# lucidrains/e2-tts-pytorch

Hardware: NVIDIA H100
Metric: mel-frames/sec E2TTS fwd+bwd (d512 depth8 L1024) (higher is better)
Workload: dtype bf16

## Files before the change

e2-tts-pytorch_b200/csrc/attn_tc.cu:

```cuda
#include <type_traits>

#include "common.cuh"
#include "ptx.cuh"

namespace b200 {

constexpr int TQ = 128, TKV = 128;
constexpr int TILE16 = 128 * 64 * 2;
constexpr int TILE8 = 64 * 64 * 2;
constexpr float LOG2E_F = 1.4426950408889634f;

struct AttnTcP {
    const unsigned int* maskbits;
    int mask_words;
    const float* gate;
    __nv_bfloat16 *o, *og;
    float* lse;
    int B, H, Np, nkv;
    float scale_over_clamp, clamp, dropout_p, keep_scale;
    unsigned int drop_thresh;
    int drop_stride;
    unsigned long long seed;
    const unsigned long long* seed_dev;
    float scale, scale_log2e;
};

__device__ __forceinline__ float tanh_approx(float x) {
    float y;
    asm("tanh.approx.f32 %0, %1;" : "=f"(y) : "f"(x));
    return y;
}
constexpr float TANH_POLY_MAX = 0.5f;
__device__ __forceinline__ float2 tanh_poly2(float2 x) {
    const float2 x2 = fmul2(x, x);
    float2 q = ffma2(x2, make_float2(62.f / 2835.f, 62.f / 2835.f), make_float2(-17.f / 315.f, -17.f / 315.f));
    q = ffma2(q, x2, make_float2(2.f / 15.f, 2.f / 15.f));
    q = ffma2(q, x2, make_float2(-1.f / 3.f, -1.f / 3.f));
    q = ffma2(q, x2, make_float2(1.f, 1.f));
    return fmul2(x, q);
}
__device__ __forceinline__ float ex2_approx(float x) {
    float y;
    asm("ex2.approx.ftz.f32 %0, %1;" : "=f"(y) : "f"(x));
    return y;
}

__global__ void attn_maskbits_kernel(const unsigned char* mask, unsigned int* bits, int B, int Np, int words) {
    const int w = blockIdx.x * blockDim.x + threadIdx.x;
    if (w >= B * words) return;
    const int b = w / words, w0 = (w % words) * 32;
    unsigned int v = 0;
    for (int i = 0; i < 32; ++i) {
        const int n = w0 + i;
        if (n < Np && (!mask || mask[(size_t)b * Np + n])) v |= 1u << i;
    }
    bits[w] = v;
}

constexpr int KV_STAGES = 3;

template <bool UNCLAMPED, int DH>
__global__ void __launch_bounds__(384, 1)
attn_fwd_wgmma_kernel(const __grid_constant__ CUtensorMap tmQ, const __grid_constant__ CUtensorMap tmK, const __grid_constant__ CUtensorMap tmV,
                      const AttnTcP p) {
    extern __shared__ uint8_t smem_raw[];
    uint8_t* smem = smem_raw + ((1024u - (smem_u32(smem_raw) & 1023u)) & 1023u);
    constexpr int NA = DH / 64;
    uint8_t* sQ = smem;
    uint8_t* sK = sQ + NA * TILE16;
    uint8_t* sV = sK + KV_STAGES * NA * TILE8;
    uint64_t* bars = reinterpret_cast<uint64_t*>(sV + KV_STAGES * NA * TILE8);
    uint64_t* q_full = bars;
    uint64_t* kv_full = bars + 1;
    uint64_t* kv_empty = bars + 4;

    const int wg = threadIdx.x >> 7;
    const int qt = blockIdx.x, hh = blockIdx.y, b = blockIdx.z;
    const int bh = b * p.H + hh;
    const int q0 = qt * TQ;
    const int nkv = (p.Np + 63) / 64;

    if (threadIdx.x == 0) {
        tma_prefetch_desc(&tmQ); tma_prefetch_desc(&tmK); tma_prefetch_desc(&tmV);
        mbar_init(q_full, 1);
        for (int i = 0; i < KV_STAGES; ++i) { mbar_init(&kv_full[i], 1); mbar_init(&kv_empty[i], 2); }
        fence_barrier_init();
    }
    __syncthreads();

    if (wg == 0) {
        regs_dealloc<40>();
        if (threadIdx.x == 0) {
            const int row_base = bh * p.Np;
            mbar_arrive_expect_tx(q_full, NA * TILE16);
#pragma unroll
            for (int a = 0; a < NA; ++a) tma_load_2d(sQ + a * TILE16, &tmQ, q_full, 64 * a, row_base + q0);
            int st = 0;
            uint32_t ph = 0;
            for (int j = 0; j < nkv; ++j) {
                mbar_wait(&kv_empty[st], ph ^ 1);
                mbar_arrive_expect_tx(&kv_full[st], 2 * NA * TILE8);
#pragma unroll
                for (int a = 0; a < NA; ++a) {
                    tma_load_2d(sK + (st * NA + a) * TILE8, &tmK, &kv_full[st], 64 * a, row_base + j * 64);
                    tma_load_2d(sV + (st * NA + a) * TILE8, &tmV, &kv_full[st], 64 * a, row_base + j * 64);
                }
                if (++st == KV_STAGES) { st = 0; ph ^= 1; }
            }
        }
        return;
    }

    regs_alloc<232>();
    const int cw = wg - 1, t = threadIdx.x & 127, lane = t & 31, wq = t >> 5;
    const int cq = 2 * (lane & 3);
    const int r0 = cw * 64 + wq * 16 + (lane >> 2);
    const unsigned int* mb = p.maskbits + (size_t)b * p.mask_words;
    const uint32_t seedmix = seed_mix32(p.seed + (p.seed_dev ? __ldg(p.seed_dev) : 0ull));
    unsigned long long drop_row[2];
#pragma unroll
    for (int i = 0; i < 2; ++i) drop_row[i] = ((unsigned long long)bh * p.Np + (unsigned long long)(q0 + r0 + 8 * i)) * (unsigned long long)p.drop_stride;
    const float2 soc2 = make_float2(p.scale_over_clamp, p.scale_over_clamp);
    const float2 cl2 = make_float2(p.clamp * LOG2E_F, p.clamp * LOG2E_F);
    const float soc = p.scale_over_clamp, soc2s = soc * soc;
    const float k1 = soc * p.clamp * LOG2E_F, k3 = k1 * soc2s * (-1.f / 3.f), k5 = k1 * soc2s * soc2s * (2.f / 15.f),
                k7 = k1 * soc2s * soc2s * soc2s * (-17.f / 315.f), k9 = k1 * soc2s * soc2s * soc2s * soc2s * (62.f / 2835.f);
    const float lim5 = 0.15f / fabsf(soc), lim9 = TANH_POLY_MAX / fabsf(soc);
    const uint32_t thr32 = drop_thresh32(p.drop_thresh);
    float l[2] = {0.f, 0.f};
    float m[2] = {-INFINITY, -INFINITY};
    float o[NA][32];
#pragma unroll
    for (int a = 0; a < NA; ++a)
#pragma unroll
        for (int i = 0; i < 32; ++i) o[a][i] = 0.f;

    mbar_wait(q_full, 0);
    const uint64_t qdesc = make_smem_desc_sw128(smem_u32(sQ + cw * TILE8), 16, 1024);
    int st = 0;
    uint32_t ph = 0;
    for (int j = 0; j < nkv; ++j) {
        mbar_wait(&kv_full[st], ph);
        float s[32];
        fence_regs(s);
        wgmma_fence();
        const uint64_t kdesc = make_smem_desc_sw128(smem_u32(sK + st * NA * TILE8), 16, 1024);
#pragma unroll
        for (int k = 0; k < DH / 16; ++k)
            wgmma_ss_n64<0, 0>(s, qdesc + (uint64_t)((k >> 2) * (TILE16 >> 4) + (k & 3) * 2), kdesc + (uint64_t)((k >> 2) * (TILE8 >> 4) + (k & 3) * 2),
                               k > 0 ? 1u : 0u);
        wgmma_commit();
        wgmma_wait<0>();
        fence_regs(s);
        if constexpr (UNCLAMPED) {
            const unsigned int mw0 = mb[2 * j], mw1 = mb[2 * j + 1];
            if ((mw0 & mw1) != 0xffffffffu) {
#pragma unroll
                for (int g = 0; g < 8; ++g) {
                    const unsigned int w = g < 4 ? mw0 : mw1;
                    const int bit = (8 * g + cq) & 31;
#pragma unroll
                    for (int i = 0; i < 2; ++i) {
                        if (!((w >> bit) & 1u)) s[4 * g + 2 * i] = -INFINITY;
                        if (!((w >> (bit + 1)) & 1u)) s[4 * g + 2 * i + 1] = -INFINITY;
                    }
                }
            }
#pragma unroll
            for (int i = 0; i < 2; ++i) {
                float tm = m[i];
#pragma unroll
                for (int g = 0; g < 8; ++g) tm = fmaxf(tm, fmaxf(s[4 * g + 2 * i], s[4 * g + 2 * i + 1]));
                tm = fmaxf(tm, __shfl_xor_sync(0xffffffffu, tm, 1));
                tm = fmaxf(tm, __shfl_xor_sync(0xffffffffu, tm, 2));
                const float mt = tm == -INFINITY ? 0.f : tm;
                const float alpha = ex2_approx((m[i] - mt) * p.scale_log2e);
                const float nm = -mt * p.scale_log2e;
                m[i] = tm;
                float ls = 0.f;
#pragma unroll
                for (int g = 0; g < 8; ++g) {
#pragma unroll
                    for (int a = 0; a < NA; ++a) {
                        o[a][4 * g + 2 * i] *= alpha;
                        o[a][4 * g + 2 * i + 1] *= alpha;
                    }
                    s[4 * g + 2 * i] = ex2_approx(__fmaf_rn(s[4 * g + 2 * i], p.scale_log2e, nm));
                    s[4 * g + 2 * i + 1] = ex2_approx(__fmaf_rn(s[4 * g + 2 * i + 1], p.scale_log2e, nm));
                    ls += s[4 * g + 2 * i] + s[4 * g + 2 * i + 1];
                }
                l[i] = __fmaf_rn(l[i], alpha, ls);
            }
        } else {
            float amax = 0.f;
#pragma unroll
            for (int i = 0; i < 32; ++i) amax = fmaxf(amax, fabsf(s[i]));
            if (__all_sync(0xffffffffu, amax <= lim5)) {
#pragma unroll
                for (int i = 0; i < 32; i += 2) {
                    const float2 x = make_float2(s[i], s[i + 1]);
                    const float2 x2 = fmul2(x, x);
                    float2 q = ffma2(x2, make_float2(k5, k5), make_float2(k3, k3));
                    q = ffma2(q, x2, make_float2(k1, k1));
                    const float2 y = fmul2(x, q);
                    s[i] = ex2_approx(y.x);
                    s[i + 1] = ex2_approx(y.y);
                }
            } else if (__all_sync(0xffffffffu, amax <= lim9)) {
#pragma unroll
                for (int i = 0; i < 32; i += 2) {
                    const float2 x = make_float2(s[i], s[i + 1]);
                    const float2 x2 = fmul2(x, x);
                    float2 q = ffma2(x2, make_float2(k9, k9), make_float2(k7, k7));
                    q = ffma2(q, x2, make_float2(k5, k5));
                    q = ffma2(q, x2, make_float2(k3, k3));
                    q = ffma2(q, x2, make_float2(k1, k1));
                    const float2 y = fmul2(x, q);
                    s[i] = ex2_approx(y.x);
                    s[i + 1] = ex2_approx(y.y);
                }
            } else {
#pragma unroll
                for (int i = 0; i < 32; ++i) {
                    const float x = s[i], x2 = x * x;
                    const float yp = x * __fmaf_rn(__fmaf_rn(__fmaf_rn(__fmaf_rn(k9, x2, k7), x2, k5), x2, k3), x2, k1);
                    const float y = fabsf(x) <= lim9 ? yp : tanh_approx(x * soc) * cl2.x;
                    s[i] = ex2_approx(y);
                }
            }
            const unsigned int mw0 = mb[2 * j], mw1 = mb[2 * j + 1];
            if ((mw0 & mw1) != 0xffffffffu) {
#pragma unroll
                for (int g = 0; g < 8; ++g) {
                    const unsigned int w = g < 4 ? mw0 : mw1;
                    const int bit = (8 * g + cq) & 31;
#pragma unroll
                    for (int i = 0; i < 2; ++i) {
                        if (!((w >> bit) & 1u)) s[4 * g + 2 * i] = 0.f;
                        if (!((w >> (bit + 1)) & 1u)) s[4 * g + 2 * i + 1] = 0.f;
                    }
                }
            }
#pragma unroll
            for (int g = 0; g < 8; ++g)
#pragma unroll
                for (int i = 0; i < 2; ++i) l[i] += s[4 * g + 2 * i] + s[4 * g + 2 * i + 1];
        }
        if (p.dropout_p > 0.f) {
#pragma unroll
            for (int g = 0; g < 8; ++g)
#pragma unroll
                for (int i = 0; i < 2; ++i) {
                    const DropWords h = drop_words(seedmix, (uint32_t)((drop_row[i] + (unsigned long long)(j * 64 + 8 * g + cq)) >> 1));
                    s[4 * g + 2 * i] = (h.a >= thr32) ? s[4 * g + 2 * i] : 0.f;
                    s[4 * g + 2 * i + 1] = (h.b >= thr32) ? s[4 * g + 2 * i + 1] : 0.f;
                }
        }
#pragma unroll
        for (int a = 0; a < NA; ++a) fence_regs(o[a]);
        wgmma_fence();
        const uint64_t vdesc = make_smem_desc_sw128(smem_u32(sV + st * NA * TILE8), 64 * 128, 1024);
#pragma unroll
        for (int kk = 0; kk < 4; ++kk) {
            const uint32_t a[4] = {pack_bf16(s[8 * kk], s[8 * kk + 1]), pack_bf16(s[8 * kk + 2], s[8 * kk + 3]),
                                   pack_bf16(s[8 * kk + 4], s[8 * kk + 5]), pack_bf16(s[8 * kk + 6], s[8 * kk + 7])};
#pragma unroll
            for (int na = 0; na < NA; ++na) wgmma_rs_n64<1>(o[na], a, vdesc + (uint64_t)(na * (TILE8 >> 4) + kk * 128), 1u);
        }
        wgmma_commit();
        wgmma_wait<0>();
#pragma unroll
        for (int a = 0; a < NA; ++a) fence_regs(o[a]);
        if (t == 0) mbar_arrive(&kv_empty[st]);
        if (++st == KV_STAGES) { st = 0; ph ^= 1; }
    }
#pragma unroll
    for (int i = 0; i < 2; ++i) {
        float lt = l[i];
        lt += __shfl_xor_sync(0xffffffffu, lt, 1);
        lt += __shfl_xor_sync(0xffffffffu, lt, 2);
        const int qi = q0 + r0 + 8 * i;
        if (qi >= p.Np) continue;
        const float inv = lt > 0.f ? p.keep_scale / lt : 0.f;
        const float gt = p.gate ? p.gate[((size_t)b * p.Np + qi) * p.H + hh] : 1.f;
        __nv_bfloat16* orow = p.o + ((size_t)bh * p.Np + qi) * DH;
        __nv_bfloat16* grow = p.og + ((size_t)b * p.Np + qi) * (size_t)(p.H * DH) + hh * DH;
#pragma unroll
        for (int a = 0; a < NA; ++a)
#pragma unroll
            for (int g = 0; g < 8; ++g) {
                const uint32_t u = pack_bf16(o[a][4 * g + 2 * i] * inv, o[a][4 * g + 2 * i + 1] * inv);
                *reinterpret_cast<uint32_t*>(orow + 64 * a + 8 * g + cq) = u;
                *reinterpret_cast<uint32_t*>(grow + 64 * a + 8 * g + cq) = pack_bf16(bf16_lo(u) * gt, bf16_hi(u) * gt);
            }
        if ((lane & 3) == 0) {
            if constexpr (UNCLAMPED) p.lse[(size_t)bh * p.Np + qi] = __fmaf_rn(m[i], p.scale, logf(lt));
            else p.lse[(size_t)bh * p.Np + qi] = logf(lt);
        }
    }
}

struct AttnBwdTcP {
    const unsigned int* maskbits; int mask_words;
    const float *lse, *delta;
    __nv_bfloat16 *dk, *dv;
    int B, H, Np, nq;
    float scale, scale_over_clamp, clamp, dropout_p, keep_scale;
    unsigned int drop_thresh; int drop_stride;
    unsigned long long seed;
    const unsigned long long* seed_dev;
    float scale_log2e;
};
constexpr int QDO_STAGES = 3, TQB = 64;
constexpr int BAR_DS_FULL = 3, BAR_DS_FREE = 5;

struct AttnPrepP {
    const float* gate;
    const __nv_bfloat16* o;
    int B, H, Np;
    const __nv_bfloat16* dog;
    float* dgate;
    __nv_bfloat16* dO_out;
    float* delta_out;
};
template <int DH>
__global__ void __launch_bounds__(256) attn_bwd_prep_kernel(const AttnPrepP p) {
    constexpr int LANES = DH / 8, LOG2_LANES = DH == 64 ? 3 : 4;
    static_assert(LANES == 1 << LOG2_LANES, "head dim 64 or 128");
    const long long gidx = (long long)blockIdx.x * 256 + threadIdx.x;
    const long long rowid = gidx >> LOG2_LANES;
    const int c = (int)(gidx & (LANES - 1));
    const long long total = (long long)p.B * p.H * p.Np;
    const bool ok = rowid < total;
    float dot = 0.f, gt = 1.f;
    long long b = 0, hh = 0, n = 0;
    if (ok) {
        n = rowid % p.Np; hh = (rowid / p.Np) % p.H; b = rowid / ((long long)p.Np * p.H);
        const uint4 dg = *reinterpret_cast<const uint4*>(p.dog + ((size_t)b * p.Np + n) * (size_t)(p.H * DH) + hh * DH + c * 8);
        const uint4 ov = *reinterpret_cast<const uint4*>(p.o + (size_t)rowid * DH + c * 8);
        gt = p.gate ? p.gate[((size_t)b * p.Np + n) * p.H + hh] : 1.f;
        const uint32_t dgv[4] = {dg.x, dg.y, dg.z, dg.w}, ovv[4] = {ov.x, ov.y, ov.z, ov.w};
        uint32_t w[4];
#pragma unroll
        for (int i = 0; i < 4; ++i) {
            const float a0 = bf16_lo(dgv[i]), a1 = bf16_hi(dgv[i]);
            dot += a0 * bf16_lo(ovv[i]) + a1 * bf16_hi(ovv[i]);
            w[i] = pack_bf16(a0 * gt, a1 * gt);
        }
        *reinterpret_cast<uint4*>(p.dO_out + (size_t)rowid * DH + c * 8) = make_uint4(w[0], w[1], w[2], w[3]);
    }
#pragma unroll
    for (int m = 1; m < LANES; m <<= 1) dot += __shfl_xor_sync(0xffffffffu, dot, m);
    if (ok && c == 0) {
        p.delta_out[rowid] = dot * gt;
        if (p.dgate) p.dgate[((size_t)b * p.Np + n) * p.H + hh] = dot;
    }
}
// ... 521 lines not shown
    const PFN_encodeTiled2 enc = tensor_map_encoder();
    B200_REQUIRE(enc, "cuTensorMapEncodeTiled entry point not available");
    B200_REQUIRE((reinterpret_cast<uintptr_t>(ptr) & 15) == 0, "attention: operand not 16-byte aligned");
    cuuint64_t gdim[2] = {(cuuint64_t)dh, (cuuint64_t)rows};
    cuuint64_t gstride[1] = {(cuuint64_t)dh * 2};
    cuuint32_t box[2] = {64, (cuuint32_t)box_rows};
    cuuint32_t estr[2] = {1, 1};
    CUresult r = enc(m, CU_TENSOR_MAP_DATA_TYPE_BFLOAT16, 2, const_cast<void*>(ptr), gdim, gstride, box, estr, CU_TENSOR_MAP_INTERLEAVE_NONE,
                     CU_TENSOR_MAP_SWIZZLE_128B, CU_TENSOR_MAP_L2_PROMOTION_L2_256B, CU_TENSOR_MAP_FLOAT_OOB_FILL_NONE);
    B200_REQUIRE(r == CUDA_SUCCESS, "cuTensorMapEncodeTiled failed (%d)", (int)r);
    return 0;
}

static int make_dq_map(CUtensorMap* m, float* dq, int BH, int Np, int dh) {
    const PFN_encodeTiled2 enc = tensor_map_encoder();
    B200_REQUIRE(enc, "cuTensorMapEncodeTiled entry point not available");
    B200_REQUIRE((reinterpret_cast<uintptr_t>(dq) & 15) == 0, "attn_bwd: dq not 16-byte aligned");
    cuuint64_t gdim[3] = {(cuuint64_t)dh, (cuuint64_t)Np, (cuuint64_t)BH};
    cuuint64_t gstride[2] = {dh * sizeof(float), (cuuint64_t)Np * dh * sizeof(float)};
    cuuint32_t box[3] = {32, TQB, 1};
    cuuint32_t estr[3] = {1, 1, 1};
    CUresult r = enc(m, CU_TENSOR_MAP_DATA_TYPE_FLOAT32, 3, dq, gdim, gstride, box, estr, CU_TENSOR_MAP_INTERLEAVE_NONE,
                     CU_TENSOR_MAP_SWIZZLE_128B, CU_TENSOR_MAP_L2_PROMOTION_L2_256B, CU_TENSOR_MAP_FLOAT_OOB_FILL_NONE);
    B200_REQUIRE(r == CUDA_SUCCESS, "cuTensorMapEncodeTiled (dq) failed (%d)", (int)r);
    return 0;
}

}

using namespace b200;

extern "C" size_t b200_attn_workspace_bytes(int32_t B, int32_t Np) {
    const int words = ((Np + 127) / 128) * 4;
    return (size_t)B * words * sizeof(unsigned int);
}

extern "C" int b200_attn_maskbits(const uint8_t* keymask, void* ws_maskbits, int32_t B, int32_t Np, b200_stream_t stream) {
    B200_REQUIRE(ws_maskbits && B > 0 && Np > 0, "attn_maskbits: bad arguments");
    const int words = ((Np + TKV - 1) / TKV) * 4;
    attn_maskbits_kernel<<<(B * words + 127) / 128, 128, 0, reinterpret_cast<cudaStream_t>(stream)>>>(
        keymask, reinterpret_cast<unsigned int*>(ws_maskbits), B, Np, words);
    return check_launch("attn_maskbits_kernel");
}

extern "C" int b200_attn_fwd(const b200_attn_fwd_args* a, b200_stream_t stream) {
    cudaStream_t st = reinterpret_cast<cudaStream_t>(stream);
    B200_REQUIRE(a && a->q && a->k && a->v && a->o && a->og && a->lse && a->ws_maskbits, "attn_fwd: null pointer");
    B200_REQUIRE(a->dim_head == 64 || a->dim_head == 128, "attn_fwd: dim_head must be 64 or 128 (got %d)", a->dim_head);
    B200_REQUIRE(a->B > 0 && a->H > 0 && a->Np > 0 && a->B <= 65535 && a->H <= 65535, "attn_fwd: bad shape");
    if (a->unclamped) {
        B200_REQUIRE(a->softclamp == 0.f, "attn_fwd: unclamped attention needs softclamp == 0 (got %g)", a->softclamp);
    } else {
        B200_REQUIRE(a->softclamp > 0.f, "attn_fwd: softclamp value must be > 0, or set unclamped for attention without the logit soft-clamp");
    }
    B200_REQUIRE(a->dropout_p >= 0.f && a->dropout_p < 1.f, "attn_fwd: dropout must be in [0,1)");
    B200_REQUIRE(a->softclamp <= 64.f, "attn_fwd: softclamp %g > 64: the clamped wgmma kernel exponentiates the clamped logits without a "
                 "running maximum, which needs exp(+-softclamp) well inside fp32 / bf16 range (the reference uses 50)", a->softclamp);
    AttnTcP p{};
    p.nkv = (a->Np + TKV - 1) / TKV;
    p.mask_words = p.nkv * 4;
    p.maskbits = reinterpret_cast<const unsigned int*>(a->ws_maskbits);
    if (!a->maskbits_ready) {
        const int total = a->B * p.mask_words;
        attn_maskbits_kernel<<<(total + 127) / 128, 128, 0, st>>>(a->keymask, reinterpret_cast<unsigned int*>(a->ws_maskbits), a->B, a->Np, p.mask_words);
        if (int rc = check_launch("attn_maskbits_kernel")) return rc;
    }
    p.gate = a->gate; p.o = (__nv_bfloat16*)a->o; p.og = (__nv_bfloat16*)a->og; p.lse = a->lse;
    p.B = a->B; p.H = a->H; p.Np = a->Np;
    if (a->unclamped) {
        p.clamp = 0.f; p.scale_over_clamp = 0.f;
    } else {
        p.clamp = a->softclamp; p.scale_over_clamp = a->scale / a->softclamp;
    }
    p.scale = a->scale; p.scale_log2e = a->scale * LOG2E_F;
    p.dropout_p = a->dropout_p;
    p.drop_thresh = (unsigned int)(a->dropout_p * 65536.f);
    p.keep_scale = 65536.f / (65536.f - (float)p.drop_thresh);
    p.seed = a->seed; p.seed_dev = reinterpret_cast<const unsigned long long*>(a->seed_dev);
    p.drop_stride = (a->Np + 1) & ~1;
    CUtensorMap tq, tk, tv;
    const long long rows = (long long)a->B * a->H * a->Np;
    const int dh = a->dim_head, na = dh / 64;
    if (make_head_map(&tq, a->q, rows, dh, 128) || make_head_map(&tk, a->k, rows, dh, 64) || make_head_map(&tv, a->v, rows, dh, 64)) return -1;
    const int smem = na * (TILE16 + 2 * KV_STAGES * TILE8) + 128 + 1024;
    static DeviceOnce once[4];
    const auto kern = dh == 64 ? (a->unclamped ? attn_fwd_wgmma_kernel<true, 64> : attn_fwd_wgmma_kernel<false, 64>)
                               : (a->unclamped ? attn_fwd_wgmma_kernel<true, 128> : attn_fwd_wgmma_kernel<false, 128>);
    cudaError_t e = set_max_smem_once(once[(a->unclamped ? 1 : 0) + (dh == 128 ? 2 : 0)], kern, smem);
    B200_REQUIRE(e == cudaSuccess, "attn_fwd: cudaFuncSetAttribute: %s", cudaGetErrorString(e));
    dim3 grid((a->Np + TQ - 1) / TQ, a->H, a->B);
    kern<<<grid, 384, smem, st>>>(tq, tk, tv, p);
    return check_launch("attn_fwd_wgmma_kernel");
}

extern "C" int b200_attn_bwd(const b200_attn_bwd_args* a, b200_stream_t stream) {
    cudaStream_t st = reinterpret_cast<cudaStream_t>(stream);
    B200_REQUIRE(a && a->q && a->k && a->v && a->o && a->d_og && a->lse && a->ws_dO && a->ws_delta && a->dq && a->dk && a->dv && a->ws_maskbits,
                 "attn_bwd: null pointer");
    B200_REQUIRE(a->dim_head == 64 || a->dim_head == 128, "attn_bwd: dim_head must be 64 or 128 (got %d)", a->dim_head);
    B200_REQUIRE(a->B > 0 && a->H > 0 && a->Np > 0 && a->B <= 65535 && a->H <= 65535, "attn_bwd: bad shape");
    if (a->unclamped) {
        B200_REQUIRE(a->softclamp == 0.f, "attn_bwd: unclamped attention needs softclamp == 0 (got %g)", a->softclamp);
    }
    B200_REQUIRE((a->unclamped || a->softclamp > 0.f) && a->dropout_p >= 0.f && a->dropout_p < 1.f, "attn_bwd: bad softclamp / dropout");
    B200_REQUIRE(a->softclamp <= 64.f, "attn_bwd: softclamp %g > 64: the clamped wgmma kernel exponentiates the clamped logits without a "
                 "running maximum, which needs exp(+-softclamp) well inside fp32 / bf16 range (the reference uses 50)", a->softclamp);
    const AttnPrepP pp{a->gate, (const __nv_bfloat16*)a->o, a->B, a->H, a->Np, (const __nv_bfloat16*)a->d_og, a->d_gate,
                       (__nv_bfloat16*)a->ws_dO, a->ws_delta};
    const int dh = a->dim_head;
    const long long prep_threads = (long long)a->B * a->H * a->Np * (dh / 8);
    if (dh == 64) attn_bwd_prep_kernel<64><<<(unsigned)((prep_threads + 255) / 256), 256, 0, st>>>(pp);
    else attn_bwd_prep_kernel<128><<<(unsigned)((prep_threads + 255) / 256), 256, 0, st>>>(pp);
    if (int rc = check_launch("attn_bwd_prep_kernel")) return rc;
    AttnBwdTcP p{};
    p.nq = (a->Np + TQB - 1) / TQB;
    p.mask_words = ((a->Np + TKV - 1) / TKV) * 4;
    p.maskbits = reinterpret_cast<const unsigned int*>(a->ws_maskbits);
    if (!a->maskbits_ready) {
        const int total = a->B * p.mask_words;
        attn_maskbits_kernel<<<(total + 127) / 128, 128, 0, st>>>(a->keymask, reinterpret_cast<unsigned int*>(a->ws_maskbits), a->B, a->Np, p.mask_words);
        if (int rc = check_launch("attn_maskbits_kernel")) return rc;
    }
    const size_t nelem = (size_t)a->B * a->H * a->Np * dh;
    cudaError_t e = cudaMemsetAsync(a->dq, 0, nelem * sizeof(float), st);
    B200_REQUIRE(e == cudaSuccess, "attn_bwd: memset: %s", cudaGetErrorString(e));
    p.lse = a->lse; p.delta = a->ws_delta;
    p.dk = (__nv_bfloat16*)a->dk; p.dv = (__nv_bfloat16*)a->dv;
    p.B = a->B; p.H = a->H; p.Np = a->Np;
    p.scale = a->scale; p.scale_log2e = a->scale * LOG2E_F;
    if (a->unclamped) {
        p.clamp = 0.f; p.scale_over_clamp = 0.f;
    } else {
        p.clamp = a->softclamp; p.scale_over_clamp = a->scale / a->softclamp;
    }
    p.dropout_p = a->dropout_p;
    p.drop_thresh = (unsigned int)(a->dropout_p * 65536.f);
    p.keep_scale = 65536.f / (65536.f - (float)p.drop_thresh);
    p.drop_stride = (a->Np + 1) & ~1;
    p.seed = a->seed; p.seed_dev = reinterpret_cast<const unsigned long long*>(a->seed_dev);
    CUtensorMap tq, tk, tv, tdo, tdq;
    const long long rows = (long long)a->B * a->H * a->Np;
    const int kv_rows = dh == 64 ? TKV : 64;
    if (make_head_map(&tq, a->q, rows, dh, TQB) || make_head_map(&tk, a->k, rows, dh, kv_rows) || make_head_map(&tv, a->v, rows, dh, kv_rows) ||
        make_head_map(&tdo, a->ws_dO, rows, dh, TQB) || make_dq_map(&tdq, reinterpret_cast<float*>(a->dq), a->B * a->H, a->Np, dh)) return -1;
    dim3 grid((a->Np + kv_rows - 1) / kv_rows, a->H, a->B);
    if (dh == 64) {
        const int smem = 2 * TILE16 + 2 * QDO_STAGES * TILE8 + 4 * TILE8 + 2 * TILE16 + 2 * 2 * 128 * (int)sizeof(float) + 128 + 1024;
        static DeviceOnce once[2];
        const auto kern = a->unclamped ? attn_bwd_wgmma_kernel<true> : attn_bwd_wgmma_kernel<false>;
        cudaError_t e2 = set_max_smem_once(once[a->unclamped ? 1 : 0], kern, smem);
        B200_REQUIRE(e2 == cudaSuccess, "attn_bwd: cudaFuncSetAttribute: %s", cudaGetErrorString(e2));
        kern<<<grid, 256, smem, st>>>(tq, tk, tv, tdo, tdq, p);
        return check_launch("attn_bwd_wgmma_kernel");
    }
    const int smem = 4 * TILE8 + 4 * QDO_STAGES * TILE8 + 2 * TILE8 + 2 * TILE16 + (2 * 16 * 128 + 2 * 128) * (int)sizeof(float) + 128 + 1024;
    static DeviceOnce once[2];
    const auto kern = a->unclamped ? attn_bwd_d128_wgmma_kernel<true> : attn_bwd_d128_wgmma_kernel<false>;
    cudaError_t e2 = set_max_smem_once(once[a->unclamped ? 1 : 0], kern, smem);
    B200_REQUIRE(e2 == cudaSuccess, "attn_bwd: cudaFuncSetAttribute: %s", cudaGetErrorString(e2));
    kern<<<grid, 256, smem, st>>>(tq, tk, tv, tdo, tdq, p);
    return check_launch("attn_bwd_d128_wgmma_kernel");
}
```

e2-tts-pytorch_b200/csrc/ptx.cuh:

```cuda
#pragma once
#include <cuda.h>
#include <cuda_bf16.h>
#include <cuda_runtime.h>
#include <stdint.h>

namespace b200 {

#ifndef B200_SPIN_LIMIT
#define B200_SPIN_LIMIT (1u << 28)
#endif

__device__ __forceinline__ uint32_t smem_u32(const void* p) { return (uint32_t)__cvta_generic_to_shared(p); }

__device__ __forceinline__ bool elect_one() {
    uint32_t pred = 0;
    asm volatile(
        "{\n\t.reg .pred P;\n\telect.sync _|P, 0xffffffff;\n\tselp.u32 %0, 1, 0, P;\n\t}\n"
        : "=r"(pred));
    return pred != 0;
}

__device__ __forceinline__ void mbar_init(uint64_t* bar, uint32_t count) {
    asm volatile("mbarrier.init.shared::cta.b64 [%0], %1;" ::"r"(smem_u32(bar)), "r"(count));
}
// ... 9 lines not shown
#ifndef B200_WAIT_HINT_NS
#define B200_WAIT_HINT_NS 0x989680u
#endif
__device__ __forceinline__ bool mbar_try_wait(uint64_t* bar, uint32_t parity) {
    uint32_t ok;
#ifdef B200_WAIT_NO_HINT
    asm volatile(
        "{\n\t.reg .pred P;\n\tmbarrier.try_wait.parity.shared::cta.b64 P, [%1], %2;\n\tselp.u32 %0, 1, 0, P;\n\t}\n"
        : "=r"(ok)
        : "r"(smem_u32(bar)), "r"(parity)
        : "memory");
#else
    asm volatile(
        "{\n\t.reg .pred P;\n\tmbarrier.try_wait.parity.shared::cta.b64 P, [%1], %2, %3;\n\tselp.u32 %0, 1, 0, P;\n\t}\n"
        : "=r"(ok)
        : "r"(smem_u32(bar)), "r"(parity), "r"(B200_WAIT_HINT_NS)
        : "memory");
#endif
    return ok != 0;
}
__device__ __forceinline__ unsigned long long global_ns() {
    unsigned long long t;
    asm volatile("mov.u64 %0, %%globaltimer;" : "=l"(t));
    return t;
}
#ifndef B200_WAIT_TIMEOUT_NS
#define B200_WAIT_TIMEOUT_NS 4000000000ull
#endif
__device__ __forceinline__ void mbar_wait(uint64_t* bar, uint32_t parity) {
    if (mbar_try_wait(bar, parity)) return;
    const unsigned long long t0 = global_ns();
    while (!mbar_try_wait(bar, parity)) {
        if (global_ns() - t0 > B200_WAIT_TIMEOUT_NS) __trap();
    }
}

__device__ __forceinline__ void tma_prefetch_desc(const CUtensorMap* m) {
    asm volatile("prefetch.tensormap [%0];" ::"l"(m) : "memory");
}
__device__ __forceinline__ void tma_load_2d(void* smem_dst, const CUtensorMap* m, uint64_t* bar, int c0, int c1) {
    asm volatile(
        "cp.async.bulk.tensor.2d.shared::cluster.global.mbarrier::complete_tx::bytes [%0], [%1, {%3, %4}], [%2];"
        ::"r"(smem_u32(smem_dst)), "l"(m), "r"(smem_u32(bar)), "r"(c0), "r"(c1)
        : "memory");
}

__device__ __forceinline__ void tma_store_2d(const CUtensorMap* m, const void* smem_src, int c0, int c1) {
    asm volatile("cp.async.bulk.tensor.2d.global.shared::cta.bulk_group [%0, {%2, %3}], [%1];"
                 ::"l"(m), "r"(smem_u32(smem_src)), "r"(c0), "r"(c1)
                 : "memory");
}
__device__ __forceinline__ void tma_reduce_add_3d(const CUtensorMap* m, const void* smem_src, int c0, int c1, int c2) {
    asm volatile("cp.reduce.async.bulk.tensor.3d.global.shared::cta.add.tile.bulk_group [%0, {%2, %3, %4}], [%1];"
                 ::"l"(m), "r"(smem_u32(smem_src)), "r"(c0), "r"(c1), "r"(c2)
                 : "memory");
}
__device__ __forceinline__ void bulk_commit_group() { asm volatile("cp.async.bulk.commit_group;" ::: "memory"); }
template <int N>
__device__ __forceinline__ void bulk_wait_group_read() { asm volatile("cp.async.bulk.wait_group.read %0;" ::"n"(N) : "memory"); }
template <int N>
__device__ __forceinline__ void bulk_wait_group() { asm volatile("cp.async.bulk.wait_group %0;" ::"n"(N) : "memory"); }
__device__ __forceinline__ void st_shared_u32(uint32_t addr, uint32_t v) { asm volatile("st.shared.b32 [%0], %1;" ::"r"(addr), "r"(v) : "memory"); }
__device__ __forceinline__ uint32_t ld_shared_u32(uint32_t addr) {
    uint32_t v;
    asm volatile("ld.shared.b32 %0, [%1];" : "=r"(v) : "r"(addr) : "memory");
    return v;
}
__device__ __forceinline__ void named_bar_sync(uint32_t id, uint32_t n) { asm volatile("bar.sync %0, %1;" ::"r"(id), "r"(n) : "memory"); }
__device__ __forceinline__ void named_bar_arrive(uint32_t id, uint32_t n) { asm volatile("bar.arrive %0, %1;" ::"r"(id), "r"(n) : "memory"); }

__device__ __forceinline__ void bulk_load_1d(void* smem_dst, const void* gsrc, uint32_t bytes, uint64_t* bar) {
    asm volatile("cp.async.bulk.shared::cluster.global.mbarrier::complete_tx::bytes [%0], [%1], %2, [%3];"
                 ::"r"(smem_u32(smem_dst)), "l"(gsrc), "r"(bytes), "r"(smem_u32(bar))
                 : "memory");
}
__device__ __forceinline__ void wgmma_fence() { asm volatile("wgmma.fence.sync.aligned;" ::: "memory"); }
__device__ __forceinline__ void wgmma_commit() { asm volatile("wgmma.commit_group.sync.aligned;" ::: "memory"); }
template <int N>
__device__ __forceinline__ void wgmma_wait() { asm volatile("wgmma.wait_group.sync.aligned %0;" ::"n"(N) : "memory"); }
template <int R>
__device__ __forceinline__ void fence_regs(float (&d)[R]) {
#pragma unroll
    for (int i = 0; i < R; ++i) asm volatile("" : "+f"(d[i])::"memory");
}
template <int N>
__device__ __forceinline__ void regs_dealloc() { asm volatile("setmaxnreg.dec.sync.aligned.u32 %0;" ::"n"(N)); }
template <int N>
__device__ __forceinline__ void regs_alloc() { asm volatile("setmaxnreg.inc.sync.aligned.u32 %0;" ::"n"(N)); }

template <int TA, int TB>
__device__ __forceinline__ void wgmma_ss_n64(float (&d)[32], uint64_t adesc, uint64_t bdesc, uint32_t accumulate) {
    asm volatile(
        "{\n\t.reg .pred p;\n\tsetp.ne.b32 p, %34, 0;\n\t"
        "wgmma.mma_async.sync.aligned.m64n64k16.f32.bf16.bf16 "
        "{%0, %1, %2, %3, %4, %5, %6, %7, %8, %9, %10, %11, %12, %13, %14, %15, %16, %17, %18, %19, %20, %21, %22, %23, %24, %25, %26, %27, %28, %29, %30, %31}, %32, %33, p, 1, 1, %35, %36;\n\t}\n"
        : "+f"(d[0]), "+f"(d[1]), "+f"(d[2]), "+f"(d[3]), "+f"(d[4]), "+f"(d[5]), "+f"(d[6]), "+f"(d[7]), "+f"(d[8]), "+f"(d[9]), "+f"(d[10]), "+f"(d[11]), "+f"(d[12]), "+f"(d[13]), "+f"(d[14]), "+f"(d[15]), "+f"(d[16]), "+f"(d[17]), "+f"(d[18]), "+f"(d[19]), "+f"(d[20]), "+f"(d[21]), "+f"(d[22]), "+f"(d[23]), "+f"(d[24]), "+f"(d[25]), "+f"(d[26]), "+f"(d[27]), "+f"(d[28]), "+f"(d[29]), "+f"(d[30]), "+f"(d[31])
        : "l"(adesc), "l"(bdesc), "r"(accumulate), "n"(TA), "n"(TB));
}

template <int TA, int TB>
__device__ __forceinline__ void wgmma_ss_n128(float (&d)[64], uint64_t adesc, uint64_t bdesc, uint32_t accumulate) {
    asm volatile(
        "{\n\t.reg .pred p;\n\tsetp.ne.b32 p, %66, 0;\n\t"
        "wgmma.mma_async.sync.aligned.m64n128k16.f32.bf16.bf16 "
        "{%0, %1, %2, %3, %4, %5, %6, %7, %8, %9, %10, %11, %12, %13, %14, %15, %16, %17, %18, %19, %20, %21, %22, %23, %24, %25, %26, %27, %28, %29, %30, %31, %32, %33, %34, %35, %36, %37, %38, %39, %40, %41, %42, %43, %44, %45, %46, %47, %48, %49, %50, %51, %52, %53, %54, %55, %56, %57, %58, %59, %60, %61, %62, %63}, %64, %65, p, 1, 1, %67, %68;\n\t}\n"
        : "+f"(d[0]), "+f"(d[1]), "+f"(d[2]), "+f"(d[3]), "+f"(d[4]), "+f"(d[5]), "+f"(d[6]), "+f"(d[7]), "+f"(d[8]), "+f"(d[9]), "+f"(d[10]), "+f"(d[11]), "+f"(d[12]), "+f"(d[13]), "+f"(d[14]), "+f"(d[15]), "+f"(d[16]), "+f"(d[17]), "+f"(d[18]), "+f"(d[19]), "+f"(d[20]), "+f"(d[21]), "+f"(d[22]), "+f"(d[23]), "+f"(d[24]), "+f"(d[25]), "+f"(d[26]), "+f"(d[27]), "+f"(d[28]), "+f"(d[29]), "+f"(d[30]), "+f"(d[31]), "+f"(d[32]), "+f"(d[33]), "+f"(d[34]), "+f"(d[35]), "+f"(d[36]), "+f"(d[37]), "+f"(d[38]), "+f"(d[39]), "+f"(d[40]), "+f"(d[41]), "+f"(d[42]), "+f"(d[43]), "+f"(d[44]), "+f"(d[45]), "+f"(d[46]), "+f"(d[47]), "+f"(d[48]), "+f"(d[49]), "+f"(d[50]), "+f"(d[51]), "+f"(d[52]), "+f"(d[53]), "+f"(d[54]), "+f"(d[55]), "+f"(d[56]), "+f"(d[57]), "+f"(d[58]), "+f"(d[59]), "+f"(d[60]), "+f"(d[61]), "+f"(d[62]), "+f"(d[63])
        : "l"(adesc), "l"(bdesc), "r"(accumulate), "n"(TA), "n"(TB));
}

template <int TA, int TB>
__device__ __forceinline__ void wgmma_ss_n256(float (&d)[128], uint64_t adesc, uint64_t bdesc, uint32_t accumulate) {
    asm volatile(
        "{\n\t.reg .pred p;\n\tsetp.ne.b32 p, %130, 0;\n\t"
        "wgmma.mma_async.sync.aligned.m64n256k16.f32.bf16.bf16 "
        "{%0, %1, %2, %3, %4, %5, %6, %7, %8, %9, %10, %11, %12, %13, %14, %15, %16, %17, %18, %19, %20, %21, %22, %23, %24, %25, %26, %27, %28, %29, %30, %31, %32, %33, %34, %35, %36, %37, %38, %39, %40, %41, %42, %43, %44, %45, %46, %47, %48, %49, %50, %51, %52, %53, %54, %55, %56, %57, %58, %59, %60, %61, %62, %63, %64, %65, %66, %67, %68, %69, %70, %71, %72, %73, %74, %75, %76, %77, %78, %79, %80, %81, %82, %83, %84, %85, %86, %87, %88, %89, %90, %91, %92, %93, %94, %95, %96, %97, %98, %99, %100, %101, %102, %103, %104, %105, %106, %107, %108, %109, %110, %111, %112, %113, %114, %115, %116, %117, %118, %119, %120, %121, %122, %123, %124, %125, %126, %127}, %128, %129, p, 1, 1, %131, %132;\n\t}\n"
        : "+f"(d[0]), "+f"(d[1]), "+f"(d[2]), "+f"(d[3]), "+f"(d[4]), "+f"(d[5]), "+f"(d[6]), "+f"(d[7]), "+f"(d[8]), "+f"(d[9]), "+f"(d[10]), "+f"(d[11]), "+f"(d[12]), "+f"(d[13]), "+f"(d[14]), "+f"(d[15]), "+f"(d[16]), "+f"(d[17]), "+f"(d[18]), "+f"(d[19]), "+f"(d[20]), "+f"(d[21]), "+f"(d[22]), "+f"(d[23]), "+f"(d[24]), "+f"(d[25]), "+f"(d[26]), "+f"(d[27]), "+f"(d[28]), "+f"(d[29]), "+f"(d[30]), "+f"(d[31]), "+f"(d[32]), "+f"(d[33]), "+f"(d[34]), "+f"(d[35]), "+f"(d[36]), "+f"(d[37]), "+f"(d[38]), "+f"(d[39]), "+f"(d[40]), "+f"(d[41]), "+f"(d[42]), "+f"(d[43]), "+f"(d[44]), "+f"(d[45]), "+f"(d[46]), "+f"(d[47]), "+f"(d[48]), "+f"(d[49]), "+f"(d[50]), "+f"(d[51]), "+f"(d[52]), "+f"(d[53]), "+f"(d[54]), "+f"(d[55]), "+f"(d[56]), "+f"(d[57]), "+f"(d[58]), "+f"(d[59]), "+f"(d[60]), "+f"(d[61]), "+f"(d[62]), "+f"(d[63]), "+f"(d[64]), "+f"(d[65]), "+f"(d[66]), "+f"(d[67]), "+f"(d[68]), "+f"(d[69]), "+f"(d[70]), "+f"(d[71]), "+f"(d[72]), "+f"(d[73]), "+f"(d[74]), "+f"(d[75]), "+f"(d[76]), "+f"(d[77]), "+f"(d[78]), "+f"(d[79]), "+f"(d[80]), "+f"(d[81]), "+f"(d[82]), "+f"(d[83]), "+f"(d[84]), "+f"(d[85]), "+f"(d[86]), "+f"(d[87]), "+f"(d[88]), "+f"(d[89]), "+f"(d[90]), "+f"(d[91]), "+f"(d[92]), "+f"(d[93]), "+f"(d[94]), "+f"(d[95]), "+f"(d[96]), "+f"(d[97]), "+f"(d[98]), "+f"(d[99]), "+f"(d[100]), "+f"(d[101]), "+f"(d[102]), "+f"(d[103]), "+f"(d[104]), "+f"(d[105]), "+f"(d[106]), "+f"(d[107]), "+f"(d[108]), "+f"(d[109]), "+f"(d[110]), "+f"(d[111]), "+f"(d[112]), "+f"(d[113]), "+f"(d[114]), "+f"(d[115]), "+f"(d[116]), "+f"(d[117]), "+f"(d[118]), "+f"(d[119]), "+f"(d[120]), "+f"(d[121]), "+f"(d[122]), "+f"(d[123]), "+f"(d[124]), "+f"(d[125]), "+f"(d[126]), "+f"(d[127])
        : "l"(adesc), "l"(bdesc), "r"(accumulate), "n"(TA), "n"(TB));
}

template <int TB>
__device__ __forceinline__ void wgmma_rs_n64(float (&d)[32], const uint32_t (&a)[4], uint64_t bdesc, uint32_t accumulate) {
    asm volatile(
        "{\n\t.reg .pred p;\n\tsetp.ne.b32 p, %37, 0;\n\t"
        "wgmma.mma_async.sync.aligned.m64n64k16.f32.bf16.bf16 "
        "{%0, %1, %2, %3, %4, %5, %6, %7, %8, %9, %10, %11, %12, %13, %14, %15, %16, %17, %18, %19, %20, %21, %22, %23, %24, %25, %26, %27, %28, %29, %30, %31}, {%32, %33, %34, %35}, %36, p, 1, 1, %38;\n\t}\n"
        : "+f"(d[0]), "+f"(d[1]), "+f"(d[2]), "+f"(d[3]), "+f"(d[4]), "+f"(d[5]), "+f"(d[6]), "+f"(d[7]), "+f"(d[8]), "+f"(d[9]), "+f"(d[10]), "+f"(d[11]), "+f"(d[12]), "+f"(d[13]), "+f"(d[14]), "+f"(d[15]), "+f"(d[16]), "+f"(d[17]), "+f"(d[18]), "+f"(d[19]), "+f"(d[20]), "+f"(d[21]), "+f"(d[22]), "+f"(d[23]), "+f"(d[24]), "+f"(d[25]), "+f"(d[26]), "+f"(d[27]), "+f"(d[28]), "+f"(d[29]), "+f"(d[30]), "+f"(d[31])
        : "r"(a[0]), "r"(a[1]), "r"(a[2]), "r"(a[3]), "l"(bdesc), "r"(accumulate), "n"(TB));
}


__device__ __forceinline__ uint64_t make_smem_desc_sw128(uint32_t smem_addr, uint32_t lbo_bytes, uint32_t sbo_bytes) {
    uint64_t d = 0;
    d |= (uint64_t)((smem_addr >> 4) & 0x3FFF);
    d |= (uint64_t)((lbo_bytes >> 4) & 0x3FFF) << 16;
    d |= (uint64_t)((sbo_bytes >> 4) & 0x3FFF) << 32;
    d |= (uint64_t)1 << 62;
    return d;
}

__device__ __forceinline__ float2 ffma2(float2 a, float2 b, float2 c) { return make_float2(__fmaf_rn(a.x, b.x, c.x), __fmaf_rn(a.y, b.y, c.y)); }
__device__ __forceinline__ float2 fmul2(float2 a, float2 b) { return make_float2(__fmul_rn(a.x, b.x), __fmul_rn(a.y, b.y)); }
__device__ __forceinline__ float2 fadd2(float2 a, float2 b) { return make_float2(__fadd_rn(a.x, b.x), __fadd_rn(a.y, b.y)); }

__device__ __forceinline__ void red_add_v4(float* p, float a, float b, float c, float d) {
    asm volatile("red.global.add.v4.f32 [%0], {%1, %2, %3, %4};" ::"l"(p), "f"(a), "f"(b), "f"(c), "f"(d) : "memory");
}
__device__ __forceinline__ void warp_red_rows_f32(float* stg, const float (&v)[32], float* base, long long ld, int row0, int nrows_total,
                                                  int ncols_valid, int lane) {
    __syncwarp();
#pragma unroll
    for (int g = 0; g < 8; ++g)
        *reinterpret_cast<float4*>(stg + lane * 32 + ((g ^ (lane & 7)) << 2)) = make_float4(v[4 * g], v[4 * g + 1], v[4 * g + 2], v[4 * g + 3]);
    __syncwarp();
    if (((ld & 3) == 0) && ((reinterpret_cast<uintptr_t>(base) & 15) == 0)) {
        const int g = lane & 7, cg = g * 4, rsub = lane >> 3;
#pragma unroll
        for (int it = 0; it < 8; ++it) {
            const int r = it * 4 + rsub;
            if (row0 + r < nrows_total) {
                const float4 s4 = *reinterpret_cast<const float4*>(stg + r * 32 + ((g ^ (r & 7)) << 2));
                float* dst = base + (long long)(row0 + r) * ld + cg;
                if (cg + 4 <= ncols_valid) red_add_v4(dst, s4.x, s4.y, s4.z, s4.w);
                else {
                    const float sp[4] = {s4.x, s4.y, s4.z, s4.w};
                    for (int j = 0; j < 4; ++j)
                        if (cg + j < ncols_valid) atomicAdd(dst + j, sp[j]);
// ... 47 lines not shown
```

Measured before the change: 335,400.

## Software-pipeline attention forward: overlap next QK^T wgmma with current PV and softmax

Restructures the forward attention consumer loop so the QK^T wgmma for tile j+1 is issued together with the PV wgmma for tile j. The softmax of the next tile then runs while the PV product is still in flight, using double-buffered packed bf16 P registers. The O rescale is deferred until after the PV wait, and the kv_empty barrier offset is generalised to the stage count. This hides tensor-core latency behind exp/mask work, but raises register pressure and adds more complex phase and stage bookkeeping.

```diff
diff --git a/e2-tts-pytorch_b200/csrc/attn_tc.cu b/e2-tts-pytorch_b200/csrc/attn_tc.cu
--- a/e2-tts-pytorch_b200/csrc/attn_tc.cu
+++ b/e2-tts-pytorch_b200/csrc/attn_tc.cu
@@ -57,7 +57,8 @@
     bits[w] = v;
 }
 
-constexpr int KV_STAGES = 3;
+template <int DH>
+constexpr int FWD_KV_STAGES = 3;
 
 template <bool UNCLAMPED, int DH>
 __global__ void __launch_bounds__(384, 1)
@@ -66,13 +67,14 @@
     extern __shared__ uint8_t smem_raw[];
     uint8_t* smem = smem_raw + ((1024u - (smem_u32(smem_raw) & 1023u)) & 1023u);
     constexpr int NA = DH / 64;
+    constexpr int KV_STAGES = FWD_KV_STAGES<DH>;
     uint8_t* sQ = smem;
     uint8_t* sK = sQ + NA * TILE16;
     uint8_t* sV = sK + KV_STAGES * NA * TILE8;
     uint64_t* bars = reinterpret_cast<uint64_t*>(sV + KV_STAGES * NA * TILE8);
     uint64_t* q_full = bars;
     uint64_t* kv_full = bars + 1;
-    uint64_t* kv_empty = bars + 4;
+    uint64_t* kv_empty = bars + 1 + KV_STAGES;
 
     const int wg = threadIdx.x >> 7;
     const int qt = blockIdx.x, hh = blockIdx.y, b = blockIdx.z;
@@ -137,23 +139,27 @@
 
     mbar_wait(q_full, 0);
     const uint64_t qdesc = make_smem_desc_sw128(smem_u32(sQ + cw * TILE8), 16, 1024);
-    int st = 0;
-    uint32_t ph = 0;
-    for (int j = 0; j < nkv; ++j) {
-        mbar_wait(&kv_full[st], ph);
-        float s[32];
-        fence_regs(s);
-        wgmma_fence();
-        const uint64_t kdesc = make_smem_desc_sw128(smem_u32(sK + st * NA * TILE8), 16, 1024);
+    auto issue_s = [&](float (&s)[32], int stg) {
+        const uint64_t kdesc = make_smem_desc_sw128(smem_u32(sK + stg * NA * TILE8), 16, 1024);
 #pragma unroll
         for (int k = 0; k < DH / 16; ++k)
             wgmma_ss_n64<0, 0>(s, qdesc + (uint64_t)((k >> 2) * (TILE16 >> 4) + (k & 3) * 2), kdesc + (uint64_t)((k >> 2) * (TILE8 >> 4) + (k & 3) * 2),
                                k > 0 ? 1u : 0u);
         wgmma_commit();
-        wgmma_wait<0>();
-        fence_regs(s);
+    };
+    auto issue_pv = [&](const uint32_t (&pk)[16], int stg) {
+        const uint64_t vdesc = make_smem_desc_sw128(smem_u32(sV + stg * NA * TILE8), 64 * 128, 1024);
+#pragma unroll
+        for (int kk = 0; kk < 4; ++kk) {
+            const uint32_t a[4] = {pk[4 * kk], pk[4 * kk + 1], pk[4 * kk + 2], pk[4 * kk + 3]};
+#pragma unroll
+            for (int na = 0; na < NA; ++na) wgmma_rs_n64<1>(o[na], a, vdesc + (uint64_t)(na * (TILE8 >> 4) + kk * 128), 1u);
+        }
+        wgmma_commit();
+    };
+    auto score = [&](float (&s)[32], int jj, uint32_t (&pk)[16], float (&alpha)[2]) {
         if constexpr (UNCLAMPED) {
-            const unsigned int mw0 = mb[2 * j], mw1 = mb[2 * j + 1];
+            const unsigned int mw0 = mb[2 * jj], mw1 = mb[2 * jj + 1];
             if ((mw0 & mw1) != 0xffffffffu) {
 #pragma unroll
                 for (int g = 0; g < 8; ++g) {
@@ -174,22 +180,17 @@
                 tm = fmaxf(tm, __shfl_xor_sync(0xffffffffu, tm, 1));
                 tm = fmaxf(tm, __shfl_xor_sync(0xffffffffu, tm, 2));
                 const float mt = tm == -INFINITY ? 0.f : tm;
-                const float alpha = ex2_approx((m[i] - mt) * p.scale_log2e);
+                alpha[i] = ex2_approx((m[i] - mt) * p.scale_log2e);
                 const float nm = -mt * p.scale_log2e;
                 m[i] = tm;
                 float ls = 0.f;
 #pragma unroll
                 for (int g = 0; g < 8; ++g) {
-#pragma unroll
-                    for (int a = 0; a < NA; ++a) {
-                        o[a][4 * g + 2 * i] *= alpha;
-                        o[a][4 * g + 2 * i + 1] *= alpha;
-                    }
                     s[4 * g + 2 * i] = ex2_approx(__fmaf_rn(s[4 * g + 2 * i], p.scale_log2e, nm));
                     s[4 * g + 2 * i + 1] = ex2_approx(__fmaf_rn(s[4 * g + 2 * i + 1], p.scale_log2e, nm));
                     ls += s[4 * g + 2 * i] + s[4 * g + 2 * i + 1];
                 }
-                l[i] = __fmaf_rn(l[i], alpha, ls);
+                l[i] = __fmaf_rn(l[i], alpha[i], ls);
             }
         } else {
             float amax = 0.f;
@@ -228,7 +229,7 @@
                     s[i] = ex2_approx(y);
                 }
             }
-            const unsigned int mw0 = mb[2 * j], mw1 = mb[2 * j + 1];
+            const unsigned int mw0 = mb[2 * jj], mw1 = mb[2 * jj + 1];
             if ((mw0 & mw1) != 0xffffffffu) {
 #pragma unroll
                 for (int g = 0; g < 8; ++g) {
@@ -251,28 +252,94 @@
             for (int g = 0; g < 8; ++g)
 #pragma unroll
                 for (int i = 0; i < 2; ++i) {
-                    const DropWords h = drop_words(seedmix, (uint32_t)((drop_row[i] + (unsigned long long)(j * 64 + 8 * g + cq)) >> 1));
+                    const DropWords h = drop_words(seedmix, (uint32_t)((drop_row[i] + (unsigned long long)(jj * 64 + 8 * g + cq)) >> 1));
                     s[4 * g + 2 * i] = (h.a >= thr32) ? s[4 * g + 2 * i] : 0.f;
                     s[4 * g + 2 * i + 1] = (h.b >= thr32) ? s[4 * g + 2 * i + 1] : 0.f;
                 }
         }
 #pragma unroll
+        for (int i = 0; i < 16; ++i) pk[i] = pack_bf16(s[2 * i], s[2 * i + 1]);
+    };
+    auto rescale = [&](const float (&alpha)[2]) {
+#pragma unroll
+        for (int g = 0; g < 8; ++g)
+#pragma unroll
+            for (int i = 0; i < 2; ++i)
+#pragma unroll
+                for (int a = 0; a < NA; ++a) {
+                    o[a][4 * g + 2 * i] *= alpha[i];
+                    o[a][4 * g + 2 * i + 1] *= alpha[i];
+                }
+    };
+
+    uint32_t pa[16], pb[16];
+    float alpha[2];
+    int st = 0;
+    uint32_t ph = 0;
+    {
+        float s[32];
+        mbar_wait(&kv_full[0], 0);
+        fence_regs(s);
+        wgmma_fence();
+        issue_s(s, 0);
+        wgmma_wait<0>();
+        fence_regs(s);
+        score(s, 0, pa, alpha);
+        if constexpr (UNCLAMPED) rescale(alpha);
+    }
+    auto step = [&](int j, uint32_t (&pcur)[16], uint32_t (&pnext)[16]) {
+        const int st1 = st + 1 == KV_STAGES ? 0 : st + 1;
+        const uint32_t ph1 = st1 == 0 ? ph ^ 1 : ph;
+        float s[32];
+        mbar_wait(&kv_full[st1], ph1);
+        fence_regs(s);
+#pragma unroll
         for (int a = 0; a < NA; ++a) fence_regs(o[a]);
         wgmma_fence();
-        const uint64_t vdesc = make_smem_desc_sw128(smem_u32(sV + st * NA * TILE8), 64 * 128, 1024);
-#pragma unroll
-        for (int kk = 0; kk < 4; ++kk) {
-            const uint32_t a[4] = {pack_bf16(s[8 * kk], s[8 * kk + 1]), pack_bf16(s[8 * kk + 2], s[8 * kk + 3]),
-                                   pack_bf16(s[8 * kk + 4], s[8 * kk + 5]), pack_bf16(s[8 * kk + 6], s[8 * kk + 7])};
-#pragma unroll
-            for (int na = 0; na < NA; ++na) wgmma_rs_n64<1>(o[na], a, vdesc + (uint64_t)(na * (TILE8 >> 4) + kk * 128), 1u);
-        }
-        wgmma_commit();
+        issue_s(s, st1);
+        issue_pv(pcur, st);
+        wgmma_wait<1>();
+        fence_regs(s);
+        score(s, j + 1, pnext, alpha);
         wgmma_wait<0>();
+        fence_regs(pcur);
 #pragma unroll
         for (int a = 0; a < NA; ++a) fence_regs(o[a]);
         if (t == 0) mbar_arrive(&kv_empty[st]);
-        if (++st == KV_STAGES) { st = 0; ph ^= 1; }
+        if constexpr (UNCLAMPED) rescale(alpha);
+        st = st1;
+        ph = ph1;
+    };
+    auto last_pv = [&](uint32_t (&pcur)[16]) {
+#pragma unroll
+        for (int a = 0; a < NA; ++a) fence_regs(o[a]);
+        wgmma_fence();
+        issue_pv(pcur, st);
+        wgmma_wait<0>();
+        fence_regs(pcur);
+#pragma unroll
+        for (int a = 0; a < NA; ++a) fence_regs(o[a]);
+        if (t == 0) mbar_arrive(&kv_empty[st]);
+    };
+    if constexpr (DH == 64) {
+        int j = 0;
+        for (; j + 2 < nkv; j += 2) {
+            step(j, pa, pb);
+            step(j + 1, pb, pa);
+        }
+        if (j + 1 < nkv) {
+            step(j, pa, pb);
+            last_pv(pb);
+        } else {
+            last_pv(pa);
+        }
+    } else {
+        for (int j = 0; j + 1 < nkv; ++j) {
+            step(j, pa, pb);
+#pragma unroll
+            for (int i = 0; i < 16; ++i) pa[i] = pb[i];
+        }
+        last_pv(pa);
     }
 #pragma unroll
     for (int i = 0; i < 2; ++i) {
@@ -960,7 +1027,8 @@
     const long long rows = (long long)a->B * a->H * a->Np;
     const int dh = a->dim_head, na = dh / 64;
     if (make_head_map(&tq, a->q, rows, dh, 128) || make_head_map(&tk, a->k, rows, dh, 64) || make_head_map(&tv, a->v, rows, dh, 64)) return -1;
-    const int smem = na * (TILE16 + 2 * KV_STAGES * TILE8) + 128 + 1024;
+    const int stages = dh == 64 ? FWD_KV_STAGES<64> : FWD_KV_STAGES<128>;
+    const int smem = na * (TILE16 + 2 * stages * TILE8) + 128 + 1024;
     static DeviceOnce once[4];
     const auto kern = dh == 64 ? (a->unclamped ? attn_fwd_wgmma_kernel<true, 64> : attn_fwd_wgmma_kernel<false, 64>)
                                : (a->unclamped ? attn_fwd_wgmma_kernel<true, 128> : attn_fwd_wgmma_kernel<false, 128>);
diff --git a/e2-tts-pytorch_b200/csrc/ptx.cuh b/e2-tts-pytorch_b200/csrc/ptx.cuh
--- a/e2-tts-pytorch_b200/csrc/ptx.cuh
+++ b/e2-tts-pytorch_b200/csrc/ptx.cuh
@@ -115,6 +115,11 @@
 __device__ __forceinline__ void fence_regs(float (&d)[R]) {
 #pragma unroll
     for (int i = 0; i < R; ++i) asm volatile("" : "+f"(d[i])::"memory");
+}
+template <int R>
+__device__ __forceinline__ void fence_regs(uint32_t (&d)[R]) {
+#pragma unroll
+    for (int i = 0; i < R; ++i) asm volatile("" : "+r"(d[i])::"memory");
 }
 template <int N>
 __device__ __forceinline__ void regs_dealloc() { asm volatile("setmaxnreg.dec.sync.aligned.u32 %0;" ::"n"(N)); }
```

After: 337,500, median of 6. Within noise of the previous version (+0.6%).
